# muzishen/RCDMs

Hardware: AMD Instinct MI355X
Metric: story-frames/sec (stage-2 UNet, 50-step DDIM, 512^2) (higher is better)
Workload: dtype f16; 1 GPU; PororoSV stage-2, 512x512, 50-step DDIM, CFG 2.0, batch=1 story x 5 frames per GPU, ctx 85x768, random-init 1276.9M-param UNet3D; stories_per_gpu=1, latent=64, ddim_steps=50, parallelism=story-replicas x1

## Files before the change

### include/rcdm.h

```cpp
#ifndef RCDM_H
#define RCDM_H

#include <stddef.h>
#include <stdint.h>

#ifdef __cplusplus
extern "C" {
#endif

#define RCDM_VERSION 0x000300

#define RCDM_OK 0
#define RCDM_EINVAL (-1)
#define RCDM_ESHAPE (-2)
#define RCDM_ELAUNCH (-3)
#define RCDM_EWORKSPACE (-4)
#define RCDM_ECOMM (-5)

#define RCDM_EPI_BIAS 1
#define RCDM_EPI_ROWVEC 2
#define RCDM_EPI_RESIDUAL 4
#define RCDM_EPI_GELU 16
#define RCDM_EPI_GEGLU 8
#define RCDM_EPI_QUICK_GELU 32
// ... 78 lines not shown
                 const float* rowvec, const void* residual, void* out, void* workspace,
                 size_t workspace_bytes, void* stream);
int rcdm_conv3x3_add1x1(const rcdm_conv3x3_desc* d, const void* in, const void* in2, const void* W, const float* bias,
                        const float* rowvec, const void* residual, void* out, void* workspace,
                        size_t workspace_bytes, void* stream);

typedef struct {
  int32_t samples, rows_per_sample, C, groups;
  int32_t ldx, ldy;
  float eps;
  int32_t silu;
} rcdm_groupnorm_desc;

size_t rcdm_groupnorm_workspace_bytes(const rcdm_groupnorm_desc* d);
int rcdm_groupnorm_silu(const rcdm_groupnorm_desc* d, const void* x, const float* gamma,
                        const float* beta, void* y, void* workspace, size_t workspace_bytes,
                        void* stream);
int rcdm_gemm_gnstat_ok(const rcdm_gemm_desc* d, const rcdm_groupnorm_desc* gn);
int rcdm_gemm_gnstat(const rcdm_gemm_desc* d, const rcdm_groupnorm_desc* gn, const void* A, const void* W, const float* bias,
                     const float* rowvec, const void* residual, void* out, void* workspace, size_t workspace_bytes,
                     void* gn_workspace, size_t gn_workspace_bytes, void* stream);
int rcdm_conv3x3_gnstat_ok(const rcdm_conv3x3_desc* d, const rcdm_groupnorm_desc* gn);
int rcdm_conv3x3_gnstat(const rcdm_conv3x3_desc* d, const rcdm_groupnorm_desc* gn, const void* in, const void* W,
                        const float* bias, const float* rowvec, const void* residual, void* out, void* workspace,
                        size_t workspace_bytes, void* gn_workspace, size_t gn_workspace_bytes, void* stream);
int rcdm_conv3x3_add1x1_gnstat(const rcdm_conv3x3_desc* d, const rcdm_groupnorm_desc* gn, const void* in, const void* in2,
                               const void* W, const float* bias, const float* rowvec, const void* residual, void* out,
                               void* workspace, size_t workspace_bytes, void* gn_workspace, size_t gn_workspace_bytes,
                               void* stream);
int rcdm_groupnorm_prestat_ok(const rcdm_groupnorm_desc* d);
int rcdm_groupnorm_silu_prestat(const rcdm_groupnorm_desc* d, const void* x, const float* gamma, const float* beta, void* y,
                                void* workspace, size_t workspace_bytes, void* stream);
int rcdm_set_groupnorm_fold(int32_t on);
int rcdm_groupnorm_stats(const rcdm_groupnorm_desc* d, const void* x, float* stat, void* workspace,
                         size_t workspace_bytes, void* stream);
int rcdm_groupnorm_stats_prestat(const rcdm_groupnorm_desc* d, float* stat, void* workspace, size_t workspace_bytes,
                                 void* stream);
int rcdm_groupnorm_finalize(int32_t samples, int32_t groups, int32_t splits, float eps, const float* partial, float* stat,
                            void* stream);
int rcdm_groupnorm_apply(const rcdm_groupnorm_desc* d, const void* x, const float* stat, const float* gamma, const float* beta,
                         void* y, void* stream);

int rcdm_conv3x3_wino_supported(const rcdm_conv3x3_desc* d);
size_t rcdm_conv3x3_wino_workspace_bytes(const rcdm_conv3x3_desc* d);
int rcdm_conv3x3_wino_plan_query(const rcdm_conv3x3_desc* d, int32_t* out8);
int rcdm_pack_conv3x3_wino(const float* w, int32_t c_out, int32_t c_in, void* dst, void* stream);
int rcdm_upsample_taps_gather(const void* P, int32_t ldp, int32_t n_img, int32_t h, int32_t w, int32_t c_out, const float* bias,
                              void* out, int32_t ldc, void* stream);
int rcdm_conv_taps_gather(const void* P, int32_t ldp, int32_t n_img, int32_t h, int32_t w, int32_t c_out, int32_t upsample,
                          const float* bias, void* out, int32_t ldc, void* stream);
int rcdm_set_wino_slab_f16(int32_t on);
int rcdm_conv3x3_wino(const rcdm_conv3x3_desc* d, const rcdm_groupnorm_desc* gn, const float* gn_stat,
                      const float* gn_gamma, const float* gn_beta, const void* in, const void* in2, const void* U,
                      const void* W2, const float* bias, const float* rowvec, const void* residual, void* out,
                      void* workspace, size_t workspace_bytes, const rcdm_groupnorm_desc* gn_out, float* gn_out_partial,
                      void* stream);

typedef struct {
  int32_t M, C, ldx, ldy;
  float eps;
  int32_t rows_per_frame, frames;
} rcdm_layernorm_desc;

int rcdm_layernorm(const rcdm_layernorm_desc* d, const void* x, const float* gamma,
                   const float* beta, const float* pe, void* y, void* stream);

#define RCDM_ATTN_WIDE_RANGE 1
typedef struct {
  int32_t batch, heads, Lq, Lk, d;
  int32_t ldq, ldk, ldv, ldo;
  float scale;
  int32_t flags;
} rcdm_attn_desc;

int rcdm_flash_attn(const rcdm_attn_desc* d, const void* Q, const void* K, const void* V, void* out,
                    void* stream);
int rcdm_flash_attn_masked(const rcdm_attn_desc* d, const void* Q, const void* K, const void* V,
                           const unsigned char* key_valid, int32_t causal, void* out, void* stream);

size_t rcdm_xattn_image_bytes(int32_t batch, int32_t heads, int32_t d);
int rcdm_xattn_pack_kv(const void* K, const void* V, int32_t batch, int32_t Lk, int32_t heads, int32_t d, int32_t ldk,
                       int32_t ldv, void* image, void* stream);
int rcdm_xattn(const rcdm_attn_desc* d, const void* Q, const void* image, void* out, void* stream);

typedef struct {
  int32_t samples, frames, pixels, heads, d;
  int32_t ldqkv, ldo;
  float scale;
} rcdm_temporal_attn_desc;

int rcdm_temporal_attn(const rcdm_temporal_attn_desc* d, const void* qkv, void* out, void* stream);

typedef struct {
  int32_t M, C;
  int32_t ldx, ldo;
  float eps;
} rcdm_ff_desc;
size_t rcdm_ff_stream_bytes(int32_t C);
int rcdm_ff_fused_supported(int32_t C);
int rcdm_pack_ff_stream(const float* w1, const float* b1, const float* w2, int32_t C, void* wstream, float* b1_packed,
                        void* stream);
int rcdm_ff_fused(const rcdm_ff_desc* d, const void* x, const float* ln_gamma, const float* ln_beta, const void* wstream,
                  const float* b1_packed, const float* b2, void* out, void* stream);

typedef struct {
  int32_t M, C;
  int32_t lda, ldr, ldt, ldo;
  int32_t tail;
  int32_t rows_per_frame, frames;
  float eps;
  int32_t gn_groups, gn_rows;
  int32_t ldz;
} rcdm_rowchain_desc;
int rcdm_rowchain_supported(int32_t C);
int rcdm_rowchain_config_supported(int32_t C, int32_t tail, int32_t pe_frames);
size_t rcdm_rowchain_stream_bytes(int32_t C, int32_t tail);
int rcdm_pack_rowchain(const float* wa, int32_t C, int32_t tail, const float* wt, const float* w1, const float* b1,
                       const float* w2, void* wstream, float* b1_packed, void* stream);
int rcdm_rowchain(const rcdm_rowchain_desc* d, const void* a_in, const void* res, void* tok, const float* a_bias,
                  const float* ln_gamma, const float* ln_beta, const float* pe, const void* wstream, const float* b1_packed,
                  const float* b2, void* out, const float* gn_stat, const float* gn_gamma, const float* gn_beta,
                  const void* z_res, const float* z_bias, void* stream);

int rcdm_softmax_rows(int32_t M, int32_t N, int32_t ldx, int32_t ldy, float scale, const void* x, void* y, void* stream);
// ... 204 lines not shown
```

### rcdms_amd/csrc/attn.hip

```cpp
#include <stdlib.h>
#include "common.h"
#include "attn_wide.h"

long long* g_attn_trace = nullptr;

namespace {

constexpr int KT = 64;

struct AttnArgs {
  const f16* Q;
  const f16* K;
  const f16* V;
  f16* O;
  int batch, heads, Lq, Lk, d, dch;
  int ldq, ldk, ldv, ldo;
  float c;
  const unsigned char* kvalid;
  int causal;
  int plain_order;
  int wide;
  long long* trace;
};

// ... 665 lines not shown
    const float inv = __builtin_amdgcn_rcpf(sum);
    for (int c = sub * 8; c < p.d; c += 8 * p.g) {
      float o[8];
#pragma unroll
      for (int e = 0; e < 8; ++e) o[e] = 0.f;
#pragma unroll
      for (int j = 0; j < F; ++j) {
        Pack16 vv;
        vv.u = *(const uint4*)(base + (size_t)j * C3 + 2 * C + c);
        const float pj = s[j] * inv;
#pragma unroll
        for (int e = 0; e < 8; ++e) o[e] = fmaf(pj, (float)vv.e[e], o[e]);
      }
      Pack16 ov;
#pragma unroll
      for (int e = 0; e < 8; ++e) ov.e[e] = (f16)o[e];
      *(uint4*)(qrow + c) = ov.u;
    }
  }
  __syncthreads();

  const int outc = C / 8;
  for (int r = wave; r < nrows; r += 4) {
    const int f = r % F, pl = r / F;
    const int px = (int)px0 + pl;
    if (px < (int)total_px) {
      const int b = px / p.pixels, pix = px - b * p.pixels;
      f16* dst = p.out + ((long)(b * F + f) * p.pixels + pix) * (long)p.ldo;
      const f16* srow = tile + (size_t)r * C3;
      for (int c = lane; c < outc; c += 64) *(uint4*)(dst + c * 8) = *(const uint4*)(srow + c * 8);
    }
  }
}

}

extern "C" {

int rcdm_flash_attn_masked(const rcdm_attn_desc* d, const void* Q, const void* K, const void* V,
                           const unsigned char* key_valid, int32_t causal, void* out, void* stream_) {
  if (!d || !Q || !K || !V || !out) return RCDM_EINVAL;
  if (d->batch <= 0 || d->heads <= 0 || d->Lq <= 0 || d->Lk <= 0 || d->d <= 0) return RCDM_EINVAL;
  const bool wide_head = d->d > 160;
  if (wide_head ? (d->d > 512 || (d->d & 63) || key_valid || causal) : (d->d & 7) != 0) return RCDM_ESHAPE;
  if ((d->ldq & 7) || (d->ldk & 7) || (d->ldv & 7) || (d->ldo & 3)) return RCDM_ESHAPE;
  if ((size_t)(d->Lk + 4 * 64) * (size_t)(d->ldk > d->ldv ? d->ldk : d->ldv) * 2 >= 0x7FFFFFFFull) return RCDM_ESHAPE;
  if (wide_head) {
    if ((size_t)d->Lq * (size_t)(d->ldq > d->ldo ? d->ldq : d->ldo) * 2 >= 0x7FFFFFFFull) return RCDM_ESHAPE;
    const int xcd_mode = attn_xcd_mode();
    AttnWideArgs w;
    w.Q = (const f16*)Q; w.K = (const f16*)K; w.V = (const f16*)V; w.O = (f16*)out;
    w.batch = d->batch; w.heads = d->heads; w.Lq = d->Lq; w.Lk = d->Lk; w.d = d->d;
    w.ldq = d->ldq; w.ldk = d->ldk; w.ldv = d->ldv; w.ldo = d->ldo;
    w.c = d->scale * 1.4426950408889634f;
    w.plain_order = xcd_mode ? 0 : 1;
    return rcdm_attn_wide_launch(w, (hipStream_t)stream_);
  }
  AttnArgs a;
  a.Q = (const f16*)Q; a.K = (const f16*)K; a.V = (const f16*)V; a.O = (f16*)out;
  a.batch = d->batch; a.heads = d->heads; a.Lq = d->Lq; a.Lk = d->Lk; a.d = d->d; a.dch = d->d / 8;
  a.ldq = d->ldq; a.ldk = d->ldk; a.ldv = d->ldv; a.ldo = d->ldo;
  a.c = d->scale * 1.4426950408889634f;
  a.kvalid = key_valid;
  a.wide = (d->flags & RCDM_ATTN_WIDE_RANGE) != 0;
  a.causal = causal ? 1 : 0;
  a.trace = g_attn_trace;
// ... 57 lines not shown
  const int DF_ = (DS + 1) / 2;
  static const int nw_mode = rcdm_env_int("RCDM_XATTN_WAVES", 4);
  const int nw = nw_mode == 8 ? 8 : 4;
  static const int qi_mode = rcdm_env_int("RCDM_XATTN_QI", 0);
  const int nqb = (d->Lq + nw * 32 - 1) / (nw * 32);
  int qi = qi_mode > 0 ? qi_mode : 1;
  if (qi_mode <= 0) {
    const int cus = rcdm_num_cus();
    const int cap = nw == 8 ? 4 : 2;
    while (qi < cap && d->batch * d->heads * ((nqb + 2 * qi - 1) / (2 * qi)) >= cus) qi *= 2;
  }
  if (qi > nqb) qi = nqb;
  if (DS > 3) qi = 1;
  a.qi = qi;
  const dim3 grid((unsigned)(d->batch * d->heads * ((nqb + qi - 1) / qi))), block(nw * 64);
  const size_t lds = (size_t)(3 * DS + 6 * DF_) * 1024;
  hipStream_t stream = (hipStream_t)stream_;
#define XA_LAUNCH(DS_)                                                                \
  if (nw == 4)                                                                        \
    hipLaunchKernelGGL((xattn_kernel<DS_, 4>), grid, block, lds, stream, a);          \
  else                                                                                \
    hipLaunchKernelGGL((xattn_kernel<DS_, 8>), grid, block, lds, stream, a)
  switch (DS) {
    case 1: XA_LAUNCH(1); break;
    case 2: XA_LAUNCH(2); break;
    case 3: XA_LAUNCH(3); break;
    case 5: XA_LAUNCH(5); break;
    default: XA_LAUNCH(10); break;
  }
#undef XA_LAUNCH
  return rcdm_check_launch();
}

int rcdm_temporal_attn(const rcdm_temporal_attn_desc* d, const void* qkv, void* out, void* stream_) {
  if (!d || !qkv || !out) return RCDM_EINVAL;
  if (d->samples <= 0 || d->pixels <= 0 || d->heads <= 0 || d->d <= 0) return RCDM_EINVAL;
  if (d->frames < 1 || d->frames > 8 || (d->d & 7) || (d->ldqkv & 7) || (d->ldo & 7)) return RCDM_ESHAPE;
  TAttnArgs a;
  a.qkv = (const f16*)qkv; a.out = (f16*)out; a.samples = d->samples; a.pixels = d->pixels;
  a.heads = d->heads; a.d = d->d; a.ldqkv = d->ldqkv; a.ldo = d->ldo; a.scale = d->scale;
  const int C = d->heads * d->d;
  const size_t px_bytes = (size_t)d->frames * 3 * C * sizeof(f16);
  static const int lds_cap_kb = rcdm_env_int("RCDM_TATTN_KB", 32);
  int tpb = (int)(((size_t)lds_cap_kb * 1024) / px_bytes);
  const int by_threads = 256 / (d->heads * d->frames);
  if (tpb > by_threads) tpb = by_threads;
  if (tpb < 1) tpb = 1;
  if ((size_t)tpb * px_bytes > 160 * 1024 || d->heads * d->frames > 256) return RCDM_ESHAPE;
  a.tpb = tpb;
  int g = 8;
  while (g > 1 && (tpb * d->heads * d->frames * g > 256 || d->d / 8 < g)) g >>= 1;
  a.g = g;
  const size_t lds = (size_t)tpb * px_bytes;
  hipStream_t stream = (hipStream_t)stream_;
  const long total_px = (long)d->samples * d->pixels;
  dim3 grid((unsigned)((total_px + tpb - 1) / tpb)), block(256);
#define TA_LAUNCH(F)                                                                                              \
  {                                                                                                               \
    static size_t lds_set = 0;                                                                                    \
    if (lds > lds_set) {                                                                                          \
      (void)hipFuncSetAttribute((const void*)temporal_attn_kernel<F>, hipFuncAttributeMaxDynamicSharedMemorySize, \
                                (int)lds);                                                                        \
      lds_set = lds;                                                                                              \
    }                                                                                                             \
    hipLaunchKernelGGL(temporal_attn_kernel<F>, grid, block, lds, stream, a);                                     \
  }
  switch (d->frames) {
    case 1: TA_LAUNCH(1); break;
    case 2: TA_LAUNCH(2); break;
    case 3: TA_LAUNCH(3); break;
    case 4: TA_LAUNCH(4); break;
    case 5: TA_LAUNCH(5); break;
    case 6: TA_LAUNCH(6); break;
    case 7: TA_LAUNCH(7); break;
    default: TA_LAUNCH(8); break;
  }
#undef TA_LAUNCH
  return rcdm_check_launch();
}

}
```

### rcdms_amd/csrc/norm.hip

```cpp
#include <stdlib.h>
#include "common.h"
#include "gn_plan.h"

namespace {

int g_gn_fold_mode = -1;

__global__ void gn_stats_kernel(const GnArgs p) {
  extern __shared__ __attribute__((aligned(16))) char smem[];
  float* part = (float*)smem;
  const int t = threadIdx.x;
  const int ch = t % p.CH, rl = t / p.CH;
  const int s = blockIdx.y, sp = blockIdx.x;
  const int r_begin = sp * p.rows_per_split;
  const int r_end = min(p.P, r_begin + p.rows_per_split);
  f32x2 S2[4], Q2[4], k2[4];
#pragma unroll
  for (int j = 0; j < 4; ++j) S2[j] = Q2[j] = k2[j] = f32x2{0.f, 0.f};
  const f16* base = p.x + (size_t)s * p.P * p.ldx + ch * 8;
  for (int r = r_begin + rl; r < r_end; r += GN_U * p.RPB) {
    Pack16 v[GN_U];
#pragma unroll
    for (int u = 0; u < GN_U; ++u) {
      const int ru = r + u * p.RPB;
// ... 151 lines not shown
  f16* yb = p.y + (size_t)s * p.P * p.ldy + ch * 8;
  const int rstep = gridDim.x * p.RPB;
  for (int r = blockIdx.x * p.RPB + rl; r < p.P; r += 4 * rstep) {
    Pack16 v[4];
#pragma unroll
    for (int u = 0; u < 4; ++u)
      if (r + u * rstep < p.P) v[u].u = *(const uint4*)(xb + (size_t)(r + u * rstep) * p.ldx);
#pragma unroll
    for (int u = 0; u < 4; ++u) {
      if (r + u * rstep >= p.P) break;
      Pack16 o;
#pragma unroll
      for (int e = 0; e < 8; ++e) {
        float f = __builtin_fmaf((float)v[u].e[e], sc[e], sh[e]);
        if (p.silu) f = silu_f(f);
        o.e[e] = (f16)f;
      }
      *(uint4*)(yb + (size_t)(r + u * rstep) * p.ldy) = o.u;
    }
  }
}

struct GnFusedArgs {
  const f16* x;
  f16* y;
  const float* gamma;
  const float* beta;
  int P, cg, GB, NCHK, RPB, ldx, ldy, silu;
  float eps;
  float* stat_out;
  int G;
};

__global__ __launch_bounds__(256) void gn_fused_kernel(const GnFusedArgs p) {
  __shared__ float part[256 * 16];
  __shared__ float gstat[16 * 2];
  const int t = threadIdx.x;
  const int ch = t % p.NCHK, rl = t / p.NCHK;
  const bool live = rl < p.RPB;
  const int s = blockIdx.y, c0 = blockIdx.x * p.GB * p.cg;
  const f16* xb = p.x + (size_t)s * p.P * p.ldx + c0 + ch * 8;
  f16* yb = p.y + (size_t)s * p.P * p.ldy + c0 + ch * 8;
  f32x2 S2[4], Q2[4], k2[4];
#pragma unroll
  for (int j = 0; j < 4; ++j) S2[j] = Q2[j] = k2[j] = f32x2{0.f, 0.f};
  if (live) {
    for (int r = rl; r < p.P; r += 4 * p.RPB) {
      Pack16 v[4];
#pragma unroll
      for (int u = 0; u < 4; ++u) {
        const int ru = r + u * p.RPB;
        v[u].u = *(const uint4*)(xb + (size_t)(ru < p.P ? ru : rl) * p.ldx);
      }
      if (r == rl) {
#pragma unroll
        for (int j = 0; j < 4; ++j) k2[j] = f32x2{(float)v[0].e[2 * j], (float)v[0].e[2 * j + 1]};
      }
#pragma unroll
      for (int u = 0; u < 4; ++u)
#pragma unroll
        for (int j = 0; j < 4; ++j) {
          const f32x2 d = f32x2{(float)v[u].e[2 * j], (float)v[u].e[2 * j + 1]} - k2[j];
          S2[j] += d;
          Q2[j] = __builtin_elementwise_fma(d, d, Q2[j]);
        }
    }
  }
  float S[8], Q[8], k[8];
#pragma unroll
  for (int j = 0; j < 4; ++j) {
    S[2 * j] = S2[j].x; S[2 * j + 1] = S2[j].y;
    Q[2 * j] = Q2[j].x; Q[2 * j + 1] = Q2[j].y;
    k[2 * j] = k2[j].x; k[2 * j + 1] = k2[j].y;
  }
  {
    const float m = live ? gn_rows_of(rl, p.P, p.RPB) : 0.f;
#pragma unroll
    for (int e = 0; e < 8; ++e) gn_shifted_moments(S[e], Q[e], k[e], m, part[t * 16 + e], part[t * 16 + 8 + e]);
  }
  __syncthreads();
  __shared__ float colsum[32 * 16];
  gn_column_moments(part, colsum, p.NCHK, p.RPB, p.P, t, 256);
  __syncthreads();
  if (t < p.GB) {
    float mean, m2;
    gn_group_moments([&](int c) { return colsum[(c >> 3) * 16 + (c & 7)]; }, [&](int c) { return colsum[(c >> 3) * 16 + 8 + (c & 7)]; },
                     t * p.cg, p.cg, (float)p.P, mean, m2);
    const float n = (float)p.P * (float)p.cg;
    gstat[t * 2] = mean;
    gstat[t * 2 + 1] = rsqrtf(m2 / n + p.eps);
    if (p.stat_out) {
      float* o = p.stat_out + ((size_t)s * p.G + blockIdx.x * p.GB + t) * 2;
      o[0] = gstat[t * 2];
      o[1] = gstat[t * 2 + 1];
    }
  }
  if (p.stat_out) return;
  __syncthreads();
  if (!live) return;
  float sc[8], sh[8];
  {
    const f32x4 g0 = *(const f32x4*)(p.gamma + c0 + ch * 8), g1 = *(const f32x4*)(p.gamma + c0 + ch * 8 + 4);
    const f32x4 b0 = *(const f32x4*)(p.beta + c0 + ch * 8), b1 = *(const f32x4*)(p.beta + c0 + ch * 8 + 4);
#pragma unroll
    for (int e = 0; e < 8; ++e) {
      const int g = (ch * 8 + e) / p.cg;
      const float mean = gstat[g * 2], rstd = gstat[g * 2 + 1];
      const float ga = e < 4 ? g0[e & 3] : g1[e & 3], be = e < 4 ? b0[e & 3] : b1[e & 3];
      sc[e] = rstd * ga;
      sh[e] = __builtin_fmaf(-(mean * rstd), ga, be);
    }
  }
  for (int r = rl; r < p.P; r += 4 * p.RPB) {
    Pack16 v[4];
#pragma unroll
    for (int u = 0; u < 4; ++u)
      if (r + u * p.RPB < p.P) v[u].u = *(const uint4*)(xb + (size_t)(r + u * p.RPB) * p.ldx);
#pragma unroll
    for (int u = 0; u < 4; ++u) {
      if (r + u * p.RPB >= p.P) break;
      Pack16 o;
#pragma unroll
      for (int e = 0; e < 8; ++e) {
        float f = __builtin_fmaf((float)v[u].e[e], sc[e], sh[e]);
        if (p.silu) f = silu_f(f);
        o.e[e] = (f16)f;
      }
      *(uint4*)(yb + (size_t)(r + u * p.RPB) * p.ldy) = o.u;
    }
  }
}

int gn_fused_bundle(int G, int cg) {
  for (int gb = 1; gb <= 8; gb <<= 1)
    if ((gb * cg) % 8 == 0 && G % gb == 0 && gb * cg / 8 <= 32) return gb;
  return 0;
}

int gn_plan(const rcdm_groupnorm_desc* d, GnArgs& a) {
  if (d->samples <= 0 || d->rows_per_sample <= 0 || d->C <= 0 || d->groups <= 0) return RCDM_EINVAL;
  if ((d->C & 7) || (d->C % d->groups) || (d->ldx & 7) || (d->ldy & 7)) return RCDM_ESHAPE;
  if (d->groups > 64 || d->C > 8192) return RCDM_ESHAPE;
  a.samples = d->samples; a.P = d->rows_per_sample; a.C = d->C; a.G = d->groups;
  a.cg = d->C / d->groups; a.CH = d->C / 8;
  a.RPB = 256 / a.CH;
  if (a.RPB < 1) a.RPB = 1;
  if (a.CH * a.RPB < a.G) a.RPB = (a.G + a.CH - 1) / a.CH;
  a.ldx = d->ldx; a.ldy = d->ldy; a.eps = d->eps; a.silu = d->silu;
  int splits = (a.P + GN_U * a.RPB - 1) / (GN_U * a.RPB);
  const int fill = (768 + a.samples - 1) / a.samples;
  const int max_splits = (a.P + 2 * a.RPB - 1) / (2 * a.RPB);
  if (splits < fill) splits = fill < max_splits ? fill : max_splits;
  const int cap = (1024 + a.samples - 1) / a.samples;
  if (splits > cap) splits = cap;
  if (splits > 512) splits = 512;
  if (splits < 1) splits = 1;
  a.rows_per_split = (a.P + splits - 1) / splits;
  a.splits = (a.P + a.rows_per_split - 1) / a.rows_per_split;
  return RCDM_OK;
}

template <int NCH, int R>
__global__ __launch_bounds__(256) void layernorm_kernel(const f16* __restrict__ x, f16* __restrict__ y,
// ... 222 lines not shown
  static const int fused_rows = rcdm_env_int("RCDM_GN_FUSED_ROWS", 512);
  const int gb = gn_fused_bundle(a.G, a.cg);
  return fused_mode && gb && a.samples * (a.G / gb) >= 48 && a.P <= fused_rows;
}

int gn_finalize_apply(GnArgs& a, hipStream_t stream) {
  const int threads = a.CH * a.RPB;
  int& fold_mode = g_gn_fold_mode;
  if (fold_mode < 0) fold_mode = rcdm_env_int("RCDM_GN_FOLD", 0);
  const int threads64 = (threads + 63) / 64 * 64;
  const bool fold = fold_mode && a.samples >= 4 && a.splits <= 128 && a.G <= 64 && threads64 <= 1024;
  if (!fold) {
    const int nsg = a.samples * a.G;
    hipLaunchKernelGGL(gn_finalize_kernel, dim3((nsg + 3) / 4), dim3(256), 0, stream, a);
    const int rc = rcdm_check_launch();
    if (rc) return rc;
  }
  int bps = (a.P + a.RPB * 8 - 1) / (a.RPB * 8);
  const int cap = (2048 + a.samples - 1) / a.samples;
  if (bps > cap) bps = cap;
  if (bps < 1) bps = 1;
  if (fold) hipLaunchKernelGGL(gn_apply_kernel<true>, dim3(bps, a.samples), dim3(threads64), 0, stream, a);
  else hipLaunchKernelGGL(gn_apply_kernel<false>, dim3(bps, a.samples), dim3(threads), 0, stream, a);
  return rcdm_check_launch();
}

}

int rcdm_gn_plan(const rcdm_groupnorm_desc* d, GnArgs& a) { return gn_plan(d, a); }
bool rcdm_gn_three_launch(const GnArgs& a) { return !gn_single_launch(a) && a.CH * a.RPB <= 1024; }

extern "C" {

int rcdm_set_groupnorm_fold(int32_t on) {
  g_gn_fold_mode = on < 0 ? -1 : (on ? 1 : 0);
  return RCDM_OK;
}

size_t rcdm_groupnorm_workspace_bytes(const rcdm_groupnorm_desc* d) {
  GnArgs a{};
  if (!d || gn_plan(d, a)) return 0;
  return ((size_t)a.samples * a.splits * a.G * 3 + (size_t)a.samples * a.G * 2) * sizeof(float);
}

int rcdm_groupnorm_silu(const rcdm_groupnorm_desc* d, const void* x, const float* gamma, const float* beta, void* y,
                        void* workspace, size_t workspace_bytes, void* stream_) {
  if (!d || !x || !gamma || !beta || !y) return RCDM_EINVAL;
  GnArgs a{};
  int rc = gn_plan(d, a);
  if (rc) return rc;
  const size_t need = ((size_t)a.samples * a.splits * a.G * 3 + (size_t)a.samples * a.G * 2) * sizeof(float);
  if (!workspace || workspace_bytes < need) return RCDM_EWORKSPACE;
  hipStream_t stream0 = (hipStream_t)stream_;
  {
    if (gn_single_launch(a)) {
      const int gb = gn_fused_bundle(a.G, a.cg);
      GnFusedArgs f;
      f.x = (const f16*)x; f.y = (f16*)y; f.gamma = gamma; f.beta = beta;
      f.P = a.P; f.cg = a.cg; f.GB = gb; f.NCHK = gb * a.cg / 8; f.RPB = 256 / f.NCHK;
      f.ldx = a.ldx; f.ldy = a.ldy; f.silu = a.silu; f.eps = a.eps;
      f.stat_out = nullptr; f.G = a.G;
      hipLaunchKernelGGL(gn_fused_kernel, dim3(a.G / gb, a.samples), dim3(256), 0, stream0, f);
      return rcdm_check_launch();
    }
  }
  a.x = (const f16*)x; a.y = (f16*)y; a.gamma = gamma; a.beta = beta;
  a.partial = (float*)workspace;
  a.stat = a.partial + (size_t)a.samples * a.splits * a.G * 3;
  hipStream_t stream = (hipStream_t)stream_;
  const int threads = a.CH * a.RPB;
  if (threads > 1024) return RCDM_ESHAPE;
  const size_t stats_lds = (size_t)(threads + a.CH) * 16 * sizeof(float);
  if (stats_lds > 64 * 1024) {
    static bool attr_set[64] = {};
    if (rcdm_first_on_device(attr_set)) {
      (void)hipFuncSetAttribute((const void*)gn_stats_kernel, hipFuncAttributeMaxDynamicSharedMemorySize, 160 * 1024);
      }
  }
  hipLaunchKernelGGL(gn_stats_kernel, dim3(a.splits, a.samples), dim3(threads), stats_lds, stream, a);
  rc = rcdm_check_launch();
  if (rc) return rc;
  return gn_finalize_apply(a, stream);
}

int rcdm_groupnorm_prestat_ok(const rcdm_groupnorm_desc* d) {
  GnArgs a{};
  if (!d || gn_plan(d, a)) return 0;
  return rcdm_gn_three_launch(a) ? 1 : 0;
}

int rcdm_groupnorm_silu_prestat(const rcdm_groupnorm_desc* d, const void* x, const float* gamma, const float* beta, void* y,
                                void* workspace, size_t workspace_bytes, void* stream_) {
  if (!d || !x || !gamma || !beta || !y) return RCDM_EINVAL;
  GnArgs a{};
  int rc = gn_plan(d, a);
  if (rc) return rc;
  if (!rcdm_gn_three_launch(a)) return RCDM_ESHAPE;
  const size_t need = ((size_t)a.samples * a.splits * a.G * 3 + (size_t)a.samples * a.G * 2) * sizeof(float);
  if (!workspace || workspace_bytes < need) return RCDM_EWORKSPACE;
  a.x = (const f16*)x; a.y = (f16*)y; a.gamma = gamma; a.beta = beta;
  a.partial = (float*)workspace;
  a.stat = a.partial + (size_t)a.samples * a.splits * a.G * 3;
  return gn_finalize_apply(a, (hipStream_t)stream_);
}

int rcdm_groupnorm_stats(const rcdm_groupnorm_desc* d, const void* x, float* stat, void* workspace, size_t workspace_bytes,
                         void* stream_) {
  if (!d || !x || !stat) return RCDM_EINVAL;
  GnArgs a{};
  int rc = gn_plan(d, a);
  if (rc) return rc;
  const size_t need = (size_t)a.samples * a.splits * a.G * 3 * sizeof(float);
  if (!workspace || workspace_bytes < need) return RCDM_EWORKSPACE;
  hipStream_t stream = (hipStream_t)stream_;
  if (gn_single_launch(a)) {
    const int gb = gn_fused_bundle(a.G, a.cg);
    GnFusedArgs f;
    f.x = (const f16*)x; f.y = nullptr; f.gamma = nullptr; f.beta = nullptr;
    f.P = a.P; f.cg = a.cg; f.GB = gb; f.NCHK = gb * a.cg / 8; f.RPB = 256 / f.NCHK;
    f.ldx = a.ldx; f.ldy = a.ldy; f.silu = 0; f.eps = a.eps;
    f.stat_out = stat; f.G = a.G;
    hipLaunchKernelGGL(gn_fused_kernel, dim3(a.G / gb, a.samples), dim3(256), 0, stream, f);
    return rcdm_check_launch();
  }
  a.x = (const f16*)x;
  a.partial = (float*)workspace;
  a.stat = stat;
  const int threads = a.CH * a.RPB;
  if (threads > 1024) return RCDM_ESHAPE;
  const size_t stats_lds = (size_t)(threads + a.CH) * 16 * sizeof(float);
  if (stats_lds > 64 * 1024) return RCDM_ESHAPE;
  hipLaunchKernelGGL(gn_stats_kernel, dim3(a.splits, a.samples), dim3(threads), stats_lds, stream, a);
  rc = rcdm_check_launch();
  if (rc) return rc;
  hipLaunchKernelGGL(gn_finalize_kernel, dim3((a.samples * a.G + 3) / 4), dim3(256), 0, stream, a);
  return rcdm_check_launch();
}

int rcdm_groupnorm_stats_prestat(const rcdm_groupnorm_desc* d, float* stat, void* workspace, size_t workspace_bytes, void* stream_) {
  if (!d || !stat) return RCDM_EINVAL;
  GnArgs a{};
  int rc = gn_plan(d, a);
  if (rc) return rc;
  if (!rcdm_gn_three_launch(a)) return RCDM_ESHAPE;
  const size_t need = (size_t)a.samples * a.splits * a.G * 3 * sizeof(float);
  if (!workspace || workspace_bytes < need) return RCDM_EWORKSPACE;
  a.partial = (float*)workspace;
  a.stat = stat;
  hipLaunchKernelGGL(gn_finalize_kernel, dim3((a.samples * a.G + 3) / 4), dim3(256), 0, (hipStream_t)stream_, a);
  return rcdm_check_launch();
}

int rcdm_groupnorm_apply(const rcdm_groupnorm_desc* d, const void* x, const float* stat, const float* gamma, const float* beta,
                         void* y, void* stream_) {
  if (!d || !x || !stat || !gamma || !beta || !y) return RCDM_EINVAL;
  GnArgs a{};
// ... 101 lines not shown
```

### rcdms_amd/hip.py

```python
import ctypes as C
import os
import sys

import torch

_HERE = os.path.dirname(os.path.abspath(__file__))
LIB_PATH = os.environ.get("RCDM_LIB") or os.path.join(_HERE, "lib", "librcdm_hip.so")

EPI_BIAS, EPI_ROWVEC, EPI_RESIDUAL, EPI_GEGLU, EPI_GELU, EPI_QUICK_GELU = 1, 2, 4, 8, 16, 32

_ERR = {-1: "RCDM_EINVAL", -2: "RCDM_ESHAPE", -3: "RCDM_ELAUNCH", -4: "RCDM_EWORKSPACE", -5: "RCDM_ECOMM"}


class RcdmError(RuntimeError):
    pass


class GemmDesc(C.Structure):
    _fields_ = [("M", C.c_int32), ("N", C.c_int32), ("K", C.c_int32),
                ("lda", C.c_int32), ("ldc", C.c_int32), ("ldr", C.c_int32),
                ("epilogue", C.c_int32), ("rows_per_sample", C.c_int32), ("ldt", C.c_int32),
                ("out_scale", C.c_float), ("split_k", C.c_int32), ("dup_rows", C.c_int32)]


# ... 91 lines not shown
    _fields_ = [("text", C.c_uint8 * 32), ("len", C.c_int32), ("id", C.c_int32), ("special", C.c_int32), ("reserved", C.c_int32)]


class TokenizeDesc(C.Structure):
    _fields_ = [("ld", C.c_int64), ("text_bytes", C.c_int64), ("n", C.c_int32), ("max_length", C.c_int32), ("truncation", C.c_int32),
                ("bos_id", C.c_int32), ("eos_id", C.c_int32), ("pad_id", C.c_int32), ("n_added", C.c_int32),
                ("pair_slots", C.c_uint32)]


TOK_MAX_CAPTION, TOK_MAX_ADDED, TOK_MAX_ROWS, TOK_MAX_ADDED_LEN, TOK_MAX_RANK, TOK_MAX_CAPTIONS = 1024, 64, 66, 32, 1 << 22, 1 << 20
SSIM_UNIFORM7, SSIM_GAUSS11 = 0, 1
PNG_BLOCK, PNG_SLOT, PNG_ADAPTIVE = 32768, 41728, -1
PNG_RGB, PNG_BGR = 0, 1
PNG_STATUS = {1: "RCDM_PNG_EZLIB", 2: "RCDM_PNG_ETRUNC", 3: "RCDM_PNG_EBLOCK", 4: "RCDM_PNG_ESTORED", 5: "RCDM_PNG_ECODES",
              6: "RCDM_PNG_ESYMBOL", 7: "RCDM_PNG_EDISTANCE", 8: "RCDM_PNG_EOVERRUN", 9: "RCDM_PNG_EUNDERRUN",
              10: "RCDM_PNG_EADLER", 11: "RCDM_PNG_EFILTER"}
IMAGE_TILE = 32
IMAGE_U8, IMAGE_F32_NCHW, IMAGE_F16_ROWS = 0, 1, 2
FRAMES_F16_ROWS, FRAMES_F32_NCHW = 0, 1

_P, _I, _F, _SZ = C.c_void_p, C.c_int32, C.c_float, C.c_size_t
SYMBOLS = {
    "rcdm_version": (C.c_int, []),
    "rcdm_last_hip_error": (C.c_int, []),
    "rcdm_last_hip_error_string": (C.c_char_p, []),
    "rcdm_gemm_ln": (C.c_int, [C.POINTER(GemmDesc), C.POINTER(LnFuse), _P, _P, _P, _P, _P, _P]),
    "rcdm_gemm_stat_parts": (C.c_int, [C.POINTER(GemmDesc)]),
    "rcdm_gemm_lnx_stat_parts": (C.c_int, [C.POINTER(GemmDesc), _I]),
    "rcdm_gemm_lnx_parts_ok": (C.c_int, [C.POINTER(GemmDesc), _I, _I]),
    "rcdm_gemm_plan_query": (C.c_int, [C.POINTER(GemmDesc), _I, _I, C.POINTER(C.c_int32)]),
    "rcdm_conv3x3_plan_query": (C.c_int, [C.POINTER(ConvDesc), C.POINTER(C.c_int32)]),
    "rcdm_gemm_lnx_workspace_bytes": (C.c_size_t, [C.POINTER(GemmDesc), _I, _I]),
    "rcdm_set_groupnorm_fold": (C.c_int, [_I]),
    "rcdm_gemm_lnx": (C.c_int, [C.POINTER(GemmDesc), C.POINTER(Lnx), _P, _P, _P, _P, _P, _P, _P, _SZ, _P]),
    "rcdm_gemm_workspace_bytes": (_SZ, [C.POINTER(GemmDesc)]),
    "rcdm_set_igemm_variant": (C.c_int, [_I]),
    "rcdm_set_shape_rules": (C.c_int, [C.c_char_p]),
    "rcdm_set_igemm_pingpong": (C.c_int, [_I]),
    "rcdm_debug_set_igemm_trace": (C.c_int, [_P]),
    "rcdm_debug_set_attn_trace": (C.c_int, [_P]),
    "rcdm_debug_mfma_peak": (C.c_int, [C.c_int32, C.c_int32, _P, _P, _P]),
    "rcdm_gemm": (C.c_int, [C.POINTER(GemmDesc), _P, _P, _P, _P, _P, _P, _P, _SZ, _P]),
    "rcdm_conv3x3_workspace_bytes": (_SZ, [C.POINTER(ConvDesc)]),
    "rcdm_conv3x3": (C.c_int, [C.POINTER(ConvDesc), _P, _P, _P, _P, _P, _P, _P, _SZ, _P]),
    "rcdm_conv3x3_add1x1": (C.c_int, [C.POINTER(ConvDesc), _P, _P, _P, _P, _P, _P, _P, _P, _SZ, _P]),
    "rcdm_conv3x3_add1x1_gnstat": (C.c_int, [C.POINTER(ConvDesc), C.POINTER(GroupNormDesc), _P, _P, _P, _P, _P, _P, _P, _P, _SZ, _P, _SZ, _P]),
    "rcdm_groupnorm_workspace_bytes": (_SZ, [C.POINTER(GroupNormDesc)]),
    "rcdm_groupnorm_silu": (C.c_int, [C.POINTER(GroupNormDesc), _P, _P, _P, _P, _P, _SZ, _P]),
    "rcdm_groupnorm_stats": (C.c_int, [C.POINTER(GroupNormDesc), _P, _P, _P, _SZ, _P]),
    "rcdm_groupnorm_stats_prestat": (C.c_int, [C.POINTER(GroupNormDesc), _P, _P, _SZ, _P]),
    "rcdm_groupnorm_prestat_ok": (C.c_int, [C.POINTER(GroupNormDesc)]),
    "rcdm_groupnorm_silu_prestat": (C.c_int, [C.POINTER(GroupNormDesc), _P, _P, _P, _P, _P, _SZ, _P]),
    "rcdm_gemm_gnstat_ok": (C.c_int, [C.POINTER(GemmDesc), C.POINTER(GroupNormDesc)]),
    "rcdm_gemm_gnstat": (C.c_int, [C.POINTER(GemmDesc), C.POINTER(GroupNormDesc), _P, _P, _P, _P, _P, _P, _P, _SZ, _P, _SZ, _P]),
    "rcdm_conv3x3_gnstat_ok": (C.c_int, [C.POINTER(ConvDesc), C.POINTER(GroupNormDesc)]),
    "rcdm_conv3x3_gnstat": (C.c_int, [C.POINTER(ConvDesc), C.POINTER(GroupNormDesc), _P, _P, _P, _P, _P, _P, _P, _SZ, _P, _SZ, _P]),
    "rcdm_softmax_rows": (C.c_int, [_I, _I, _I, _I, C.c_float, _P, _P, _P]),
    "rcdm_layernorm": (C.c_int, [C.POINTER(LayerNormDesc), _P, _P, _P, _P, _P, _P]),
    "rcdm_flash_attn": (C.c_int, [C.POINTER(AttnDesc), _P, _P, _P, _P, _P]),
    "rcdm_flash_attn_masked": (C.c_int, [C.POINTER(AttnDesc), _P, _P, _P, _P, _I, _P, _P]),
    "rcdm_temporal_attn": (C.c_int, [C.POINTER(TemporalAttnDesc), _P, _P, _P]),
    "rcdm_ff_stream_bytes": (_SZ, [_I]),
    "rcdm_ff_fused_supported": (C.c_int, [_I]),
    "rcdm_pack_ff_stream": (C.c_int, [_P, _P, _P, _I, _P, _P, _P]),
    "rcdm_ff_fused": (C.c_int, [C.POINTER(FFDesc), _P, _P, _P, _P, _P, _P, _P, _P]),
    "rcdm_rowchain_supported": (C.c_int, [_I]),
    "rcdm_rowchain_config_supported": (C.c_int, [_I, _I, _I]),
    "rcdm_rowchain_stream_bytes": (_SZ, [_I, _I]),
    "rcdm_pack_rowchain": (C.c_int, [_P, _I, _I, _P, _P, _P, _P, _P, _P, _P]),
    "rcdm_rowchain": (C.c_int, [C.POINTER(RowChainDesc), _P, _P, _P, _P, _P, _P, _P, _P, _P, _P, _P, _P, _P, _P, _P, _P, _P]),
    "rcdm_timestep_embed": (C.c_int, [_P, _I, _I, _P, _P]),
    "rcdm_small_linear": (C.c_int, [_P, _I, _I, _P, _P, _I, _I, _I, _P, _P]),
    "rcdm_assemble_input": (C.c_int, [_P, _P, _P, _I, _I, _I, _I, _I, _P, _I, _I, _P]),
    "rcdm_ncfhw_to_rows": (C.c_int, [_P, _I, _I, _I, _I, _I, _P, _I, _I, _P]),
    "rcdm_rows_to_ncfhw": (C.c_int, [_P, _I, _I, _I, _I, _I, _I, _P, _P]),
    "rcdm_cfg_ddim_step": (C.c_int, [_P, _I, _P, _I, _I, _I, _I, _I, _F, _P, _P, _P]),
    "rcdm_cfg_pndm_step": (C.c_int, [_P, _I, _P, _P, _I, _I, _I, _I, _I, _F, _P, _P, _P]),
    "rcdm_cfg_sigma_step": (C.c_int, [_P, _I, _P, _P, _P, _P, _I, _I, _I, _I, _I, _F, _P, _P, _P]),
    "rcdm_cfg_rescale_workspace_bytes": (_SZ, [_I, _I, _I, _I]),
    "rcdm_cfg_rescale_factor": (C.c_int, [_P, _I, _I, _I, _I, _I, _F, _F, _P, _SZ, _P, _P]),
    "rcdm_cfg_ddim_step_scaled": (C.c_int, [_P, _I, _P, _I, _I, _I, _I, _I, _F, _P, _P, _P, _P]),
    "rcdm_cfg_pndm_step_scaled": (C.c_int, [_P, _I, _P, _P, _I, _I, _I, _I, _I, _F, _P, _P, _P, _P]),
    "rcdm_cfg_sigma_step_scaled": (C.c_int, [_P, _I, _P, _P, _P, _P, _I, _I, _I, _I, _I, _F, _P, _P, _P, _P]),
    "rcdm_prior_assemble": (C.c_int, [_P, _P, _P, _I, _P, _P, _I, _I, _I, _I, _I, _P]),
    "rcdm_cfg_unclip_step": (C.c_int, [_P, _I, _P, _I, _I, _I, C.c_float, C.c_float, _P, _P, _P, _P]),
    "rcdm_embed_tokens": (C.c_int, [_P, _I, _I, _P, _I, _P, _I, _P, _I, _P]),
    "rcdm_patch_rows": (C.c_int, [_P, _I, _I, _I, _I, _P, _I, _P]),
    "rcdm_load_timestep": (C.c_int, [_P, _P, _P, _I, _P]),
    "rcdm_image_resample_lds_bytes": (_SZ, [C.POINTER(ResampleDesc)]),
    "rcdm_image_resample": (C.c_int, [C.POINTER(ResampleDesc), _P, _P, _P, _P, _P, _P, _P]),
    "rcdm_frames_to_u8": (C.c_int, [C.POINTER(FramesU8Desc), _P, _P, _P]),
    "rcdm_png_bound": (_SZ, [C.POINTER(PngDesc)]),
    "rcdm_png_workspace_bytes": (_SZ, [C.POINTER(PngDesc)]),
    "rcdm_png_encode": (C.c_int, [C.POINTER(PngDesc), _P, _P, _P, _P, _P]),
# ... 163 lines not shown
                                             gn_ws_ptr, gn_ws_bytes, stream_ptr() if stream is None else stream),
           "rcdm_conv3x3_add1x1_gnstat")


def groupnorm_stats(desc, x, stat, ws_ptr, ws_bytes, stream=None):
    _check(load().rcdm_groupnorm_stats(C.byref(desc), x, stat, ws_ptr, ws_bytes,
                                       stream_ptr() if stream is None else stream), "rcdm_groupnorm_stats")


def groupnorm_stats_prestat(desc, stat, ws_ptr, ws_bytes, stream=None):
    _check(load().rcdm_groupnorm_stats_prestat(C.byref(desc), stat, ws_ptr, ws_bytes,
                                               stream_ptr() if stream is None else stream), "rcdm_groupnorm_stats_prestat")


def layernorm(desc, x, gamma, beta, pe, y, stream=None):
    _check(load().rcdm_layernorm(C.byref(desc), x, gamma, beta, pe, y,
                                 stream_ptr() if stream is None else stream), "rcdm_layernorm")


def softmax_rows(M, N, ldx, ldy, scale, x, y, stream=None):
    _check(load().rcdm_softmax_rows(M, N, ldx, ldy, scale, x, y, stream_ptr() if stream is None else stream),
           "rcdm_softmax_rows")


def gemm_ln(desc, ln, a, w, bias, residual, out, stream=None):
    _check(load().rcdm_gemm_ln(C.byref(desc), C.byref(ln), a, w, bias, residual, out,
                               stream_ptr() if stream is None else stream), "rcdm_gemm_ln")


def set_groupnorm_fold(on):
    _check(load().rcdm_set_groupnorm_fold(int(on)), "rcdm_set_groupnorm_fold")


def gemm_stat_parts(desc, consumer=False):
    if consumer:
        return int(load().rcdm_gemm_lnx_stat_parts(C.byref(desc), 1))
    return int(load().rcdm_gemm_stat_parts(C.byref(desc)))


_PLAN_FIELDS = ("variant", "bm", "bn", "tiles_m", "tiles_n", "splits", "blocks_per_cu", "k_steps")


def gemm_plan_query(desc, producer=False, consumer=False):
    out = (C.c_int32 * 8)()
    _check(load().rcdm_gemm_plan_query(C.byref(desc), int(bool(producer)), int(bool(consumer)), out), "rcdm_gemm_plan_query")
    return dict(zip(_PLAN_FIELDS, out))


def conv3x3_plan_query(desc):
    out = (C.c_int32 * 8)()
    _check(load().rcdm_conv3x3_plan_query(C.byref(desc), out), "rcdm_conv3x3_plan_query")
    return dict(zip(_PLAN_FIELDS, out))


def gemm_lnx_parts_ok(desc, parts, consumer=False):
    return bool(load().rcdm_gemm_lnx_parts_ok(C.byref(desc), int(parts), int(bool(consumer))))


def gemm_lnx_workspace_bytes(desc, producer=False, consumer=False):
    return int(load().rcdm_gemm_lnx_workspace_bytes(C.byref(desc), int(bool(producer)), int(bool(consumer))))


def gemm_lnx(desc, lnx, a, w, bias, rowvec, residual, out, workspace, workspace_bytes, stream=None):
    _check(load().rcdm_gemm_lnx(C.byref(desc), C.byref(lnx), a, w, bias, rowvec, residual, out, workspace, workspace_bytes,
                                stream_ptr() if stream is None else stream), "rcdm_gemm_lnx")


def flash_attn(desc, q, k, v, out, stream=None):
    _check(load().rcdm_flash_attn(C.byref(desc), q, k, v, out,
                                  stream_ptr() if stream is None else stream), "rcdm_flash_attn")


def flash_attn_masked(desc, q, k, v, key_valid, causal, out, stream=None):
    _check(load().rcdm_flash_attn_masked(C.byref(desc), q, k, v, key_valid, int(causal), out,
                                         stream_ptr() if stream is None else stream), "rcdm_flash_attn_masked")


def temporal_attn(desc, qkv, out, stream=None):
    _check(load().rcdm_temporal_attn(C.byref(desc), qkv, out,
                                     stream_ptr() if stream is None else stream), "rcdm_temporal_attn")


def ff_stream_bytes(Cc):
    return load().rcdm_ff_stream_bytes(Cc)


def ff_fused_supported(Cc):
    return bool(load().rcdm_ff_fused_supported(Cc))


def rowchain_supported(Cc):
    return bool(load().rcdm_rowchain_supported(Cc))


def rowchain_config_supported(Cc, tail, pe_frames=0):
    return bool(load().rcdm_rowchain_config_supported(Cc, tail, pe_frames))


def rowchain_stream_bytes(Cc, tail):
    return load().rcdm_rowchain_stream_bytes(Cc, tail)


def pack_rowchain(wa, Cc, tail, wt, w1, b1, w2, wstream, b1p, stream=None):
    _check(load().rcdm_pack_rowchain(wa, Cc, tail, wt, w1, b1, w2, wstream, b1p,
                                     stream_ptr() if stream is None else stream), "rcdm_pack_rowchain")


def rowchain(desc, a_in, res, tok, a_bias, ln_g, ln_b, pe, wstream, b1p, b2, out, stream=None, gn_stat=None, gn_g=None,
             gn_b=None, z_res=None, z_bias=None):
    _check(load().rcdm_rowchain(C.byref(desc), a_in, res, tok, a_bias, ln_g, ln_b, pe, wstream, b1p, b2, out,
                                gn_stat, gn_g, gn_b, z_res, z_bias, stream_ptr() if stream is None else stream), "rcdm_rowchain")


# ... 365 lines not shown
```

Measured before the change: 6.179 story-frames/s.

## Add register-resident temporal attention kernel and register-cached fused groupnorm

Adds a temporal attention kernel for 5 frames that keeps q/k/v for one pixel-head in registers across a 64-lane wave, with no LDS staging, and selects it by default when the head-dim/group combination matches. The fused groupnorm kernel gains templated variants that hold up to 16 rows per thread in registers, so the apply pass no longer rereads the input from memory. The aim is to cut LDS traffic, global rereads and sync cost in two memory-bound kernels. In exchange, register pressure rises, and the attention grid of small one-wave blocks may lower occupancy efficiency.

```diff
diff --git a/include/rcdm.h b/include/rcdm.h
--- a/include/rcdm.h
+++ b/include/rcdm.h
@@ -134,6 +134,7 @@
 int rcdm_groupnorm_silu_prestat(const rcdm_groupnorm_desc* d, const void* x, const float* gamma, const float* beta, void* y,
                                 void* workspace, size_t workspace_bytes, void* stream);
 int rcdm_set_groupnorm_fold(int32_t on);
+int rcdm_set_groupnorm_fused_regs(int32_t on);
 int rcdm_groupnorm_stats(const rcdm_groupnorm_desc* d, const void* x, float* stat, void* workspace,
                          size_t workspace_bytes, void* stream);
 int rcdm_groupnorm_stats_prestat(const rcdm_groupnorm_desc* d, float* stat, void* workspace, size_t workspace_bytes,
@@ -192,6 +193,8 @@
 } rcdm_temporal_attn_desc;
 
 int rcdm_temporal_attn(const rcdm_temporal_attn_desc* d, const void* qkv, void* out, void* stream);
+int rcdm_set_temporal_attn_form(int32_t form);
+int rcdm_temporal_attn_form(const rcdm_temporal_attn_desc* d);
 
 typedef struct {
   int32_t M, C;
diff --git a/rcdms_amd/csrc/attn.hip b/rcdms_amd/csrc/attn.hip
--- a/rcdms_amd/csrc/attn.hip
+++ b/rcdms_amd/csrc/attn.hip
@@ -721,6 +721,106 @@
     }
   }
 }
+
+template <int G, int NCH>
+__global__ __launch_bounds__(64) void temporal_attn_regs_kernel(const TAttnArgs p) {
+  constexpr int F = 5;
+  constexpr int PHW = 64 / (F * G);
+  const int lane = threadIdx.x;
+  const int sub = lane % G, item = lane / G;
+  const int i = item % F, phl = item / F;
+  const long total_ph = (long)p.samples * p.pixels * p.heads;
+  const long ph_ = (long)blockIdx.x * PHW + phl;
+  const bool ok = phl < PHW && ph_ < total_ph;
+  const long ph = ok ? ph_ : 0;
+  const int head = (int)(ph % p.heads);
+  const long px = ph / p.heads;
+  const int b = (int)(px / p.pixels), pix = (int)(px - (long)b * p.pixels);
+  const int C = p.heads * p.d;
+  const long fstride = (long)p.pixels * p.ldqkv;
+  const f16* base = p.qkv + ((long)b * F * p.pixels + pix) * (long)p.ldqkv + head * p.d;
+
+  int cc[NCH];
+  bool live[NCH];
+#pragma unroll
+  for (int k = 0; k < NCH; ++k) {
+    const int c = (sub + G * k) * 8;
+    live[k] = c < p.d;
+    cc[k] = live[k] ? c : p.d - 8;
+  }
+  Pack16 qv[NCH], kv[F][NCH], vv[F][NCH];
+#pragma unroll
+  for (int k = 0; k < NCH; ++k) qv[k].u = *(const uint4*)(base + i * fstride + cc[k]);
+#pragma unroll
+  for (int j = 0; j < F; ++j)
+#pragma unroll
+    for (int k = 0; k < NCH; ++k) kv[j][k].u = *(const uint4*)(base + j * fstride + C + cc[k]);
+#pragma unroll
+  for (int j = 0; j < F; ++j)
+#pragma unroll
+    for (int k = 0; k < NCH; ++k) vv[j][k].u = *(const uint4*)(base + j * fstride + 2 * C + cc[k]);
+  __builtin_amdgcn_sched_barrier(0);
+
+  float s[F];
+#pragma unroll
+  for (int j = 0; j < F; ++j) s[j] = 0.f;
+#pragma unroll
+  for (int k = 0; k < NCH; ++k) {
+#pragma unroll
+    for (int j = 0; j < F; ++j) {
+      float acc = s[j];
+#pragma unroll
+      for (int e = 0; e < 8; ++e) acc = fmaf((float)qv[k].e[e], (float)kv[j][k].e[e], acc);
+      s[j] = live[k] ? acc : s[j];
+    }
+  }
+#pragma unroll
+  for (int off = 1; off < G; off <<= 1) {
+#pragma unroll
+    for (int j = 0; j < F; ++j) s[j] += __shfl_xor(s[j], off, 64);
+  }
+  float mx = s[0] * p.scale;
+#pragma unroll
+  for (int j = 0; j < F; ++j) {
+    s[j] *= p.scale;
+    mx = fmaxf(mx, s[j]);
+  }
+  float sum = 0.f;
+#pragma unroll
+  for (int j = 0; j < F; ++j) {
+    s[j] = __expf(s[j] - mx);
+    sum += s[j];
+  }
+  const float inv = __builtin_amdgcn_rcpf(sum);
+  f16* orow = p.out + ((long)(b * F + i) * p.pixels + pix) * (long)p.ldo + head * p.d;
+#pragma unroll
+  for (int k = 0; k < NCH; ++k) {
+    float o[8];
+#pragma unroll
+    for (int e = 0; e < 8; ++e) o[e] = 0.f;
+#pragma unroll
+    for (int j = 0; j < F; ++j) {
+      const float pj = s[j] * inv;
+#pragma unroll
+      for (int e = 0; e < 8; ++e) o[e] = fmaf(pj, (float)vv[j][k].e[e], o[e]);
+    }
+    Pack16 ov;
+#pragma unroll
+    for (int e = 0; e < 8; ++e) ov.e[e] = (f16)o[e];
+    if (ok && live[k]) *(uint4*)(orow + cc[k]) = ov.u;
+  }
+}
+
+int tattn_regs_inst(int frames, int d, int g) {
+  if (frames != 5) return 0;
+  const int nch = (d / 8 + g - 1) / g;
+  if (g == 2 && nch == 3) return 1;
+  if (g == 4 && nch == 3) return 2;
+  if (g == 4 && nch == 5) return 3;
+  return 0;
+}
+
+int g_tattn_form = -2;
 
 }
 
@@ -844,13 +944,9 @@
   return rcdm_check_launch();
 }
 
-int rcdm_temporal_attn(const rcdm_temporal_attn_desc* d, const void* qkv, void* out, void* stream_) {
-  if (!d || !qkv || !out) return RCDM_EINVAL;
+static int tattn_plan(const rcdm_temporal_attn_desc* d, int* tpb_, int* g_, int* regs_inst) {
   if (d->samples <= 0 || d->pixels <= 0 || d->heads <= 0 || d->d <= 0) return RCDM_EINVAL;
   if (d->frames < 1 || d->frames > 8 || (d->d & 7) || (d->ldqkv & 7) || (d->ldo & 7)) return RCDM_ESHAPE;
-  TAttnArgs a;
-  a.qkv = (const f16*)qkv; a.out = (f16*)out; a.samples = d->samples; a.pixels = d->pixels;
-  a.heads = d->heads; a.d = d->d; a.ldqkv = d->ldqkv; a.ldo = d->ldo; a.scale = d->scale;
   const int C = d->heads * d->d;
   const size_t px_bytes = (size_t)d->frames * 3 * C * sizeof(f16);
   static const int lds_cap_kb = rcdm_env_int("RCDM_TATTN_KB", 32);
@@ -859,10 +955,46 @@
   if (tpb > by_threads) tpb = by_threads;
   if (tpb < 1) tpb = 1;
   if ((size_t)tpb * px_bytes > 160 * 1024 || d->heads * d->frames > 256) return RCDM_ESHAPE;
-  a.tpb = tpb;
   int g = 8;
   while (g > 1 && (tpb * d->heads * d->frames * g > 256 || d->d / 8 < g)) g >>= 1;
+  if (g_tattn_form == -2) g_tattn_form = rcdm_env_int("RCDM_TATTN_REGS", -1);
+  const int inst = g_tattn_form == 0 ? 0 : tattn_regs_inst(d->frames, d->d, g);
+  *tpb_ = tpb; *g_ = g; *regs_inst = inst;
+  return RCDM_OK;
+}
+
+int rcdm_set_temporal_attn_form(int32_t form) {
+  g_tattn_form = form < 0 ? -1 : (form ? 1 : 0);
+  return RCDM_OK;
+}
+
+int rcdm_temporal_attn_form(const rcdm_temporal_attn_desc* d) {
+  int tpb, g, inst;
+  if (!d || tattn_plan(d, &tpb, &g, &inst)) return -1;
+  return inst ? 1 : 0;
+}
+
+int rcdm_temporal_attn(const rcdm_temporal_attn_desc* d, const void* qkv, void* out, void* stream_) {
+  if (!d || !qkv || !out) return RCDM_EINVAL;
+  int tpb, g, inst;
+  const int prc = tattn_plan(d, &tpb, &g, &inst);
+  if (prc) return prc;
+  TAttnArgs a;
+  a.qkv = (const f16*)qkv; a.out = (f16*)out; a.samples = d->samples; a.pixels = d->pixels;
+  a.heads = d->heads; a.d = d->d; a.ldqkv = d->ldqkv; a.ldo = d->ldo; a.scale = d->scale;
+  a.tpb = tpb;
   a.g = g;
+  if (inst) {
+    const long total_ph = (long)d->samples * d->pixels * d->heads;
+    const int phw = 64 / (5 * g);
+    const dim3 rgrid((unsigned)((total_ph + phw - 1) / phw)), rblock(64);
+    hipStream_t rstream = (hipStream_t)stream_;
+    if (inst == 1) hipLaunchKernelGGL((temporal_attn_regs_kernel<2, 3>), rgrid, rblock, 0, rstream, a);
+    else if (inst == 2) hipLaunchKernelGGL((temporal_attn_regs_kernel<4, 3>), rgrid, rblock, 0, rstream, a);
+    else hipLaunchKernelGGL((temporal_attn_regs_kernel<4, 5>), rgrid, rblock, 0, rstream, a);
+    return rcdm_check_launch();
+  }
+  const size_t px_bytes = (size_t)d->frames * 3 * d->heads * d->d * sizeof(f16);
   const size_t lds = (size_t)tpb * px_bytes;
   hipStream_t stream = (hipStream_t)stream_;
   const long total_px = (long)d->samples * d->pixels;
diff --git a/rcdms_amd/csrc/norm.hip b/rcdms_amd/csrc/norm.hip
--- a/rcdms_amd/csrc/norm.hip
+++ b/rcdms_amd/csrc/norm.hip
@@ -207,6 +207,7 @@
   int G;
 };
 
+template <int NR>
 __global__ __launch_bounds__(256) void gn_fused_kernel(const GnFusedArgs p) {
   __shared__ float part[256 * 16];
   __shared__ float gstat[16 * 2];
@@ -219,7 +220,26 @@
   f32x2 S2[4], Q2[4], k2[4];
 #pragma unroll
   for (int j = 0; j < 4; ++j) S2[j] = Q2[j] = k2[j] = f32x2{0.f, 0.f};
-  if (live) {
+  Pack16 keep[NR > 0 ? NR : 1];
+  if (NR > 0 && live && rl < p.P) {
+#pragma unroll
+    for (int u = 0; u < NR; ++u) {
+      const int ru = rl + u * p.RPB;
+      keep[u].u = *(const uint4*)(xb + (size_t)(ru < p.P ? ru : rl) * p.ldx);
+    }
+    __builtin_amdgcn_sched_barrier(0);
+#pragma unroll
+    for (int j = 0; j < 4; ++j) k2[j] = f32x2{(float)keep[0].e[2 * j], (float)keep[0].e[2 * j + 1]};
+#pragma unroll
+    for (int u = 0; u < NR; ++u)
+#pragma unroll
+      for (int j = 0; j < 4; ++j) {
+        const f32x2 d = f32x2{(float)keep[u].e[2 * j], (float)keep[u].e[2 * j + 1]} - k2[j];
+        S2[j] += d;
+        Q2[j] = __builtin_elementwise_fma(d, d, Q2[j]);
+      }
+  }
+  if (NR == 0 && live) {
     for (int r = rl; r < p.P; r += 4 * p.RPB) {
       Pack16 v[4];
 #pragma unroll
@@ -286,6 +306,22 @@
       sh[e] = __builtin_fmaf(-(mean * rstd), ga, be);
     }
   }
+  if constexpr (NR > 0) {
+#pragma unroll
+    for (int u = 0; u < NR; ++u) {
+      const int ru = rl + u * p.RPB;
+      if (ru >= p.P) break;
+      Pack16 o;
+#pragma unroll
+      for (int e = 0; e < 8; ++e) {
+        float f = __builtin_fmaf((float)keep[u].e[e], sc[e], sh[e]);
+        if (p.silu) f = silu_f(f);
+        o.e[e] = (f16)f;
+      }
+      *(uint4*)(yb + (size_t)ru * p.ldy) = o.u;
+    }
+    return;
+  }
   for (int r = rl; r < p.P; r += 4 * p.RPB) {
     Pack16 v[4];
 #pragma unroll
@@ -304,6 +340,18 @@
       *(uint4*)(yb + (size_t)(r + u * p.RPB) * p.ldy) = o.u;
     }
   }
+}
+
+int g_gn_fused_regs = -1;
+
+int gn_fused_launch(const GnFusedArgs& f, dim3 grid, hipStream_t stream) {
+  if (g_gn_fused_regs < 0) g_gn_fused_regs = rcdm_env_int("RCDM_GN_FUSED_REGS", 1) ? 1 : 0;
+  const int rows = (f.P + f.RPB - 1) / f.RPB;
+  if (!g_gn_fused_regs || rows > 16) hipLaunchKernelGGL(gn_fused_kernel<0>, grid, dim3(256), 0, stream, f);
+  else if (rows <= 4) hipLaunchKernelGGL(gn_fused_kernel<4>, grid, dim3(256), 0, stream, f);
+  else if (rows <= 8) hipLaunchKernelGGL(gn_fused_kernel<8>, grid, dim3(256), 0, stream, f);
+  else hipLaunchKernelGGL(gn_fused_kernel<16>, grid, dim3(256), 0, stream, f);
+  return rcdm_check_launch();
 }
 
 int gn_fused_bundle(int G, int cg) {
@@ -592,6 +640,11 @@
 
 extern "C" {
 
+int rcdm_set_groupnorm_fused_regs(int32_t on) {
+  g_gn_fused_regs = on < 0 ? -1 : (on ? 1 : 0);
+  return RCDM_OK;
+}
+
 int rcdm_set_groupnorm_fold(int32_t on) {
   g_gn_fold_mode = on < 0 ? -1 : (on ? 1 : 0);
   return RCDM_OK;
@@ -620,8 +673,7 @@
       f.P = a.P; f.cg = a.cg; f.GB = gb; f.NCHK = gb * a.cg / 8; f.RPB = 256 / f.NCHK;
       f.ldx = a.ldx; f.ldy = a.ldy; f.silu = a.silu; f.eps = a.eps;
       f.stat_out = nullptr; f.G = a.G;
-      hipLaunchKernelGGL(gn_fused_kernel, dim3(a.G / gb, a.samples), dim3(256), 0, stream0, f);
-      return rcdm_check_launch();
+      return gn_fused_launch(f, dim3(a.G / gb, a.samples), stream0);
     }
   }
   a.x = (const f16*)x; a.y = (f16*)y; a.gamma = gamma; a.beta = beta;
@@ -680,8 +732,7 @@
     f.P = a.P; f.cg = a.cg; f.GB = gb; f.NCHK = gb * a.cg / 8; f.RPB = 256 / f.NCHK;
     f.ldx = a.ldx; f.ldy = a.ldy; f.silu = 0; f.eps = a.eps;
     f.stat_out = stat; f.G = a.G;
-    hipLaunchKernelGGL(gn_fused_kernel, dim3(a.G / gb, a.samples), dim3(256), 0, stream, f);
-    return rcdm_check_launch();
+    return gn_fused_launch(f, dim3(a.G / gb, a.samples), stream);
   }
   a.x = (const f16*)x;
   a.partial = (float*)workspace;
diff --git a/rcdms_amd/hip.py b/rcdms_amd/hip.py
--- a/rcdms_amd/hip.py
+++ b/rcdms_amd/hip.py
@@ -147,6 +147,7 @@
     "rcdm_conv3x3_plan_query": (C.c_int, [C.POINTER(ConvDesc), C.POINTER(C.c_int32)]),
     "rcdm_gemm_lnx_workspace_bytes": (C.c_size_t, [C.POINTER(GemmDesc), _I, _I]),
     "rcdm_set_groupnorm_fold": (C.c_int, [_I]),
+    "rcdm_set_groupnorm_fused_regs": (C.c_int, [_I]),
     "rcdm_gemm_lnx": (C.c_int, [C.POINTER(GemmDesc), C.POINTER(Lnx), _P, _P, _P, _P, _P, _P, _P, _SZ, _P]),
     "rcdm_gemm_workspace_bytes": (_SZ, [C.POINTER(GemmDesc)]),
     "rcdm_set_igemm_variant": (C.c_int, [_I]),
@@ -175,6 +176,8 @@
     "rcdm_flash_attn": (C.c_int, [C.POINTER(AttnDesc), _P, _P, _P, _P, _P]),
     "rcdm_flash_attn_masked": (C.c_int, [C.POINTER(AttnDesc), _P, _P, _P, _P, _I, _P, _P]),
     "rcdm_temporal_attn": (C.c_int, [C.POINTER(TemporalAttnDesc), _P, _P, _P]),
+    "rcdm_set_temporal_attn_form": (C.c_int, [_I]),
+    "rcdm_temporal_attn_form": (C.c_int, [C.POINTER(TemporalAttnDesc)]),
     "rcdm_ff_stream_bytes": (_SZ, [_I]),
     "rcdm_ff_fused_supported": (C.c_int, [_I]),
     "rcdm_pack_ff_stream": (C.c_int, [_P, _P, _P, _I, _P, _P, _P]),
@@ -404,6 +407,10 @@
     _check(load().rcdm_set_groupnorm_fold(int(on)), "rcdm_set_groupnorm_fold")
 
 
+def set_groupnorm_fused_regs(on):
+    _check(load().rcdm_set_groupnorm_fused_regs(int(on)), "rcdm_set_groupnorm_fused_regs")
+
+
 def gemm_stat_parts(desc, consumer=False):
     if consumer:
         return int(load().rcdm_gemm_lnx_stat_parts(C.byref(desc), 1))
@@ -451,6 +458,14 @@
 def temporal_attn(desc, qkv, out, stream=None):
     _check(load().rcdm_temporal_attn(C.byref(desc), qkv, out,
                                      stream_ptr() if stream is None else stream), "rcdm_temporal_attn")
+
+
+def set_temporal_attn_form(form):
+    _check(load().rcdm_set_temporal_attn_form(int(form)), "rcdm_set_temporal_attn_form")
+
+
+def temporal_attn_form(desc):
+    return int(load().rcdm_temporal_attn_form(C.byref(desc)))
 
 
 def ff_stream_bytes(Cc):
```

New measurement: 6.224 story-frames/s (median of 6 runs). Within noise of the previous version (+0.7%).
